# aluo7/ViT-SOM

Measured on AMD Instinct MI355X. Metric: images/sec/node ViT-SOM 40x40 CIFAR-10 bs512 (training step: fwd+bwd+all-reduce+AdamW), higher is better.
Workload: dtype f32 (Linear GEMMs on bf16 MFMA: forward from an exact 3xbf16 operand split, six products; weight / input gradients from a 2xbf16 split, three products, rel. error 4e-6)

## Files before the change

include/vitsom_hip.h:

```cpp
#ifndef VITSOM_HIP_H
#define VITSOM_HIP_H

#include <stddef.h>
#include <stdint.h>

#ifdef __cplusplus
extern "C" {
#endif

typedef struct ihipStream_t* vsom_stream_t;

#define VSOM_OK 0
#define VSOM_EINVAL (-1)
#define VSOM_EALIGN (-2)
#define VSOM_EUNSUPPORTED (-3)
#define VSOM_EWORKSPACE (-4)

#define VSOM_VERSION 100

#define VSOM_DIST_COSINE 0
#define VSOM_DIST_EUCLIDEAN 1
#define VSOM_DIST_MANHATTAN 2

int vsom_version(void);
// ... 70 lines not shown
                               const float* gamma, const float* resid, float* dX, int rows, int cols, void* part,
                               size_t part_bytes, vsom_stream_t stream);
int vsom_layernorm_bwd_finish_many(const int64_t* jobs_dev, int first, int count, int max_cols, vsom_stream_t stream);

int vsom_linear_bwd_input_ln_supported(int M, int N, int K);
size_t vsom_linear_bwd_input_ln_partial_bytes(int M, int K);
int vsom_linear_bwd_input_ln(const float* dY, long lddy, const float* Wt, int M, int N, int K, const float* X,
                             const float* mean, const float* rstd, const float* gamma, const float* resid, float* dX,
                             float* dgamma, float* dbeta, void* ws, size_t ws_bytes, vsom_stream_t stream);
int vsom_linear_bwd_input_ln_partial(const float* dY, long lddy, const float* Wt, int M, int N, int K, const float* X,
                                     const float* mean, const float* rstd, const float* gamma, const float* resid,
                                     float* dX, void* part, size_t part_bytes, vsom_stream_t stream);

int vsom_attention_fwd(const float* qkv, float* out, float* lse, int B, int N, int H, int hd,
                       vsom_stream_t stream);
int vsom_attention_bwd(const float* qkv, const float* out, const float* dout, const float* lse,
                       float* dqkv, float* delta_ws, int B, int N, int H, int hd,
                       vsom_stream_t stream);
int vsom_attention_probs(const float* qkv, const float* lse, float* probs, int B, int N, int H, int hd,
                         vsom_stream_t stream);
int vsom_set_attention_fused(int fused);

int vsom_attention_q1_fwd(const float* q, const float* kv, float* o, float* lse, int B, int N, int H, int hd,
                          vsom_stream_t stream);
int vsom_attention_q1_bwd(const float* dout, const float* o, const float* lse, const float* q, const float* kv, float* dq,
                          float* dkv, int B, int N, int H, int hd, vsom_stream_t stream);
int vsom_rows_add(const float* src, long lds, float* dst, long ldd, int rows, int cols, vsom_stream_t stream);

int vsom_row_inv_norm(const float* X, long ldx, int rows, int cols, float eps, float* inv_norm,
                      vsom_stream_t stream);
// ... 263 lines not shown
```

vit_som_amd/_lib.py:

```python
import ctypes as C
import os

import torch

_HERE = os.path.dirname(os.path.abspath(__file__))
LIB_PATH = os.path.join(_HERE, "libvitsom_hip.so")

c_fp = C.c_void_p
c_stream = C.c_void_p

SIGNATURES = {
    "vsom_version": (C.c_int, []),
    "vsom_last_error_string": (C.c_char_p, []),
    "vsom_linear_fwd": (C.c_int, [c_fp, C.c_long, c_fp, c_fp, c_fp, C.c_long, C.c_int, C.c_int, C.c_int, c_stream]),
    "vsom_linear_gelu_fwd": (C.c_int, [c_fp, C.c_long, c_fp, c_fp, c_fp, c_fp, C.c_int, C.c_int, C.c_int, c_stream]),
    "vsom_linear_relu_fwd": (C.c_int, [c_fp, C.c_long, c_fp, c_fp, c_fp, c_fp, C.c_int, C.c_int, C.c_int, c_stream]),
    "vsom_l1_loss_workspace_bytes": (C.c_size_t, [C.c_long]),
    "vsom_l1_loss": (C.c_int, [c_fp, c_fp, c_fp, c_fp, C.c_float, C.c_long, c_fp, C.c_size_t, c_stream]),
    "vsom_linear_residual_fwd": (C.c_int, [c_fp, C.c_long, c_fp, c_fp, c_fp, C.c_long, C.c_int, c_fp, C.c_long,
                                           C.c_int, C.c_int, C.c_int, c_stream]),
    "vsom_linear_bwd_input": (C.c_int, [c_fp, C.c_long, c_fp, c_fp, C.c_long, C.c_int, C.c_int, C.c_int, C.c_int,
                                        c_fp, c_stream]),
    "vsom_linear_bwd_input_t": (C.c_int, [c_fp, C.c_long, c_fp, c_fp, C.c_long, C.c_int, C.c_int, C.c_int, C.c_int,
                                          c_fp, c_stream]),
# ... 10 lines not shown
                                       C.c_int, c_stream]),
    "vsom_patch_embed_bwd_workspace_bytes": (C.c_size_t, [C.c_int] * 5),
    "vsom_patch_embed_bwd": (C.c_int, [c_fp, c_fp, c_fp, c_fp, c_fp, C.c_int, C.c_int, C.c_int, C.c_int, C.c_int,
                                       c_fp, C.c_size_t, c_stream]),
    "vsom_layernorm_fwd": (C.c_int, [c_fp, c_fp, c_fp, c_fp, c_fp, c_fp, C.c_int, C.c_int, C.c_float, c_stream]),
    "vsom_layernorm_bwd_workspace_bytes": (C.c_size_t, [C.c_int, C.c_int]),
    "vsom_layernorm_bwd": (C.c_int, [c_fp] * 9 + [C.c_int, C.c_int, c_fp, C.c_size_t, c_stream]),
    "vsom_layernorm_bwd_deferrable": (C.c_int, [C.c_int, C.c_int]),
    "vsom_layernorm_bwd_partial": (C.c_int, [c_fp] * 7 + [C.c_int, C.c_int, c_fp, C.c_size_t, c_stream]),
    "vsom_layernorm_bwd_finish_many": (C.c_int, [c_fp, C.c_int, C.c_int, C.c_int, c_stream]),
    "vsom_linear_bwd_input_ln_supported": (C.c_int, [C.c_int, C.c_int, C.c_int]),
    "vsom_linear_bwd_input_ln_partial_bytes": (C.c_size_t, [C.c_int, C.c_int]),
    "vsom_linear_bwd_input_ln": (C.c_int, [c_fp, C.c_long, c_fp, C.c_int, C.c_int, C.c_int] + [c_fp] * 8 + [c_fp, C.c_size_t, c_stream]),
    "vsom_linear_bwd_input_ln_partial": (C.c_int, [c_fp, C.c_long, c_fp, C.c_int, C.c_int, C.c_int] + [c_fp] * 6 + [c_fp, C.c_size_t, c_stream]),
    "vsom_attention_fwd": (C.c_int, [c_fp, c_fp, c_fp, C.c_int, C.c_int, C.c_int, C.c_int, c_stream]),
    "vsom_attention_bwd": (C.c_int, [c_fp] * 6 + [C.c_int] * 4 + [c_stream]),
    "vsom_set_attention_fused": (C.c_int, [C.c_int]),
    "vsom_attention_probs": (C.c_int, [c_fp, c_fp, c_fp, C.c_int, C.c_int, C.c_int, C.c_int, c_stream]),
    "vsom_attention_q1_fwd": (C.c_int, [c_fp] * 4 + [C.c_int] * 4 + [c_stream]),
    "vsom_attention_q1_bwd": (C.c_int, [c_fp] * 7 + [C.c_int] * 4 + [c_stream]),
    "vsom_rows_add": (C.c_int, [c_fp, C.c_long, c_fp, C.c_long, C.c_int, C.c_int, c_stream]),
    "vsom_tape_begin": (C.c_int, []),
    "vsom_tape_cut": (C.c_int, []),
    "vsom_tape_pause": (C.c_int, [C.c_int]),
    "vsom_tape_end": (C.c_int, []),
    "vsom_tape_recording": (C.c_int, []),
    "vsom_tape_segment_ops": (C.c_int, [C.c_int, C.c_int]),
    "vsom_tape_replay": (C.c_int, [C.c_int, C.c_int]),
    "vsom_tape_destroy": (C.c_int, [C.c_int]),
    "vsom_event_record": (C.c_int, [C.c_int, c_stream]),
# ... 257 lines not shown
```

vit_som_amd/csrc/attention.hip:

```cpp
#include "common.h"
#include "attention_layout.h"

#include <atomic>

#include <stdlib.h>

#pragma clang fp contract(off)

namespace vsom {

int gemm_grad_products();

static std::atomic<int> g_attn_fused{1};

#ifdef VSOM_ATTN_STAMPS
__device__ unsigned long long* g_attn_stamps = nullptr;
#define ATTN_STAMP(i)                                                                              \
    do {                                                                                           \
        if (threadIdx.x == 0 && g_attn_stamps) g_attn_stamps[blockIdx.x * 16 + (i)] = __builtin_amdgcn_s_memrealtime(); \
    } while (0)
#define ATTN_STAMP_HWID()                                                                          \
    do {                                                                                           \
        if (threadIdx.x == 0 && g_attn_stamps) {                                                   \
            unsigned hw, xcc;                                                                      \
// ... 134 lines not shown
__device__ __forceinline__ float tile_sum(float v) {
    v += dpp_row<0x128>(v); v += dpp_row<0x124>(v); v += dpp_row<0x122>(v); v += dpp_row<0x121>(v);
    return v;
}
__device__ __forceinline__ float tile_max(float v) {
    v = fmaxf(v, dpp_row<0x128>(v)); v = fmaxf(v, dpp_row<0x124>(v));
    v = fmaxf(v, dpp_row<0x122>(v)); v = fmaxf(v, dpp_row<0x121>(v));
    return v;
}
__device__ __forceinline__ float wave_sum64(float v) { return group_sum(tile_sum(v)); }
template <bool EXTRA>
__device__ __forceinline__ int tok(int t, int r) { return (EXTRA ? 1 : 0) + 16 * t + r; }

template <int HDP>
__device__ __forceinline__ void stage_rows(float* lds, const float* __restrict__ src, long rs, int N, int nrows,
                                           int hd) {
    constexpr int S = ACfg<HDP>::S;
    if constexpr (ACfg<HDP>::VEC) {
        constexpr int C4 = HDP / 4;
        for (int idx = threadIdx.x; idx < nrows * C4; idx += blockDim.x) {
            const int row = idx / C4, c4 = idx % C4;
            f32x4 v = {0.f, 0.f, 0.f, 0.f};
            if (row < N) v = *reinterpret_cast<const f32x4*>(src + (long)row * rs + 4 * c4);
            *reinterpret_cast<f32x4*>(lds + ACfg<HDP>::off(row, 4 * c4)) = v;
        }
    } else {
        for (int idx = threadIdx.x; idx < nrows * HDP; idx += blockDim.x) {
            const int row = idx / HDP, c = idx % HDP;
            lds[row * S + c] = (row < N && c < hd) ? src[(long)row * rs + c] : 0.f;
        }
    }
}
template <int HDP>
__device__ __forceinline__ void stage_rows_pair(float* ldsA, const float* __restrict__ srcA, long rsA, float* ldsB,
                                                const float* __restrict__ srcB, long rsB, int N, int nrows, int hd) {
    if constexpr (ACfg<HDP>::VEC) {
        constexpr int C4 = HDP / 4;
        const int total = nrows * C4, step = blockDim.x;
        for (int base = threadIdx.x; base < total; base += 4 * step) {
            f32x4 va[4], vb[4];
#pragma unroll
            for (int u = 0; u < 4; ++u) {
                const int idx = base + u * step, row = idx / C4, c4 = idx % C4;
                va[u] = f32x4{0.f, 0.f, 0.f, 0.f};
                vb[u] = f32x4{0.f, 0.f, 0.f, 0.f};
                if (idx < total && row < N) {
                    va[u] = *reinterpret_cast<const f32x4*>(srcA + (long)row * rsA + 4 * c4);
                    vb[u] = *reinterpret_cast<const f32x4*>(srcB + (long)row * rsB + 4 * c4);
                }
            }
#pragma unroll
            for (int u = 0; u < 4; ++u) {
                const int idx = base + u * step, row = idx / C4, c4 = idx % C4;
                if (idx < total) {
                    *reinterpret_cast<f32x4*>(ldsA + ACfg<HDP>::off(row, 4 * c4)) = va[u];
                    *reinterpret_cast<f32x4*>(ldsB + ACfg<HDP>::off(row, 4 * c4)) = vb[u];
                }
            }
        }
    } else {
        stage_rows<HDP>(ldsA, srcA, rsA, N, nrows, hd);
        stage_rows<HDP>(ldsB, srcB, rsB, N, nrows, hd);
    }
}
template <int HDP>
__device__ __forceinline__ void stage_rows_quad(float* l0, const float* __restrict__ s0, long r0, float* l1,
                                                const float* __restrict__ s1, long r1, float* l2,
                                                const float* __restrict__ s2, long r2, float* l3,
                                                const float* __restrict__ s3, long r3, int N, int nrows) {
    constexpr int C4 = HDP / 4;
    const int total = nrows * C4, step = blockDim.x;
    for (int base = threadIdx.x; base < total; base += 4 * step) {
        f32x4 v[4][4];
#pragma unroll
        for (int u = 0; u < 4; ++u) {
            const int idx = base + u * step, row = idx / C4, c4 = idx % C4;
            const bool ok = idx < total && row < N;
// ... 4 lines not shown
            v[3][u] = ok ? *reinterpret_cast<const f32x4*>(s3 + (long)row * r3 + 4 * c4) : z;
        }
#pragma unroll
        for (int u = 0; u < 4; ++u) {
            const int idx = base + u * step, row = idx / C4, c4 = idx % C4;
            if (idx < total) {
                *reinterpret_cast<f32x4*>(l0 + ACfg<HDP>::off(row, 4 * c4)) = v[0][u];
                *reinterpret_cast<f32x4*>(l1 + ACfg<HDP>::off(row, 4 * c4)) = v[1][u];
                *reinterpret_cast<f32x4*>(l2 + ACfg<HDP>::off(row, 4 * c4)) = v[2][u];
                *reinterpret_cast<f32x4*>(l3 + ACfg<HDP>::off(row, 4 * c4)) = v[3][u];
            }
        }
    }
}
template <int HDP>
__device__ __forceinline__ void stage_vec(float* lds, const float* __restrict__ src, int hd) {
    for (int c = threadIdx.x; c < HDP; c += blockDim.x) lds[c] = (c < hd) ? src[c] : 0.f;
}

template <int HDP>
__device__ __forceinline__ void load_frag(float (&f)[ACfg<HDP>::NMM], const float* rowptr, int qp, bool ok,
                                          int hd) {
    if constexpr (ACfg<HDP>::VEC) {
#pragma unroll
        for (int g = 0; g < HDP / 16; ++g) {
            f32x4 v = {0.f, 0.f, 0.f, 0.f};
            if (ok) v = *reinterpret_cast<const f32x4*>(rowptr + 16 * g + 4 * qp);
#pragma unroll
            for (int s = 0; s < 4; ++s) f[4 * g + s] = v[s];
        }
    } else {
#pragma unroll
// ... 252 lines not shown
    for (int t = 0; t < ntile; ++t) {
        f32x4 s, dp;
        score_tile2<HDP>(Qs, tok<EXTRA>(t, 0), kf, Ds, tok<EXTRA>(t, 0), vf, r, qp, s, dp);
        f32x4 p, ds;
#pragma unroll
        for (int e = 0; e < 4; ++e) {
            const int query = tok<EXTRA>(t, 4 * qp + e);
            p[e] = (EXTRA || (query < N && kok)) ? __expf(s[e] * scale - Ls[query]) : 0.f;
            ds[e] = p[e] * (dp[e] - Es[query]) * scale;
        }
        accum_tile2<HDP>(dv, Ds, p, dk, Qs, ds, tok<EXTRA>(t, 0), r, qp);
    }
}

template <int HDP, bool EXTRA>
__global__ __launch_bounds__(512, 4) void attn_fwd_kernel(const float* __restrict__ qkv, float* __restrict__ out,
                                                       float* __restrict__ lse, int N, int H, int hd,
                                                       float scale) {
    extern __shared__ __attribute__((aligned(16))) float smem[];
    constexpr int NDT = ACfg<HDP>::NDT;
    constexpr int NMM = ACfg<HDP>::NMM;
    const int b = blockIdx.x / H, h = blockIdx.x % H;
    const int E = H * hd, E3 = 3 * E;
    const int lane = threadIdx.x & 63, wave = threadIdx.x >> 6, nwaves = blockDim.x >> 6;
    const int r = lane & 15, qp = lane >> 4;
    const AttnLayout<float*> lay(smem, N, HDP, EXTRA, nwaves, ATTN_LDS_FWD);
    const int ntile = lay.ntile;
    float* Ks = lay.Y0;
    float* Vs = lay.Y1;
    float* X0 = lay.X0;
    float* PA = lay.PA;
    const float* base = qkv + (long)b * N * E3 + h * hd;
    float qf[NMM];
    ATTN_STAMP(0);
    ATTN_STAMP_HWID();
    load_frag<HDP>(qf, base + (long)tok<EXTRA>(wave, r) * E3, qp, tok<EXTRA>(wave, r) < N, hd);
    stage_rows_pair<HDP>(Ks, base + E, E3, Vs, base + 2 * E, E3, N, lay.nrows, hd);
    if (EXTRA) stage_vec<HDP>(X0, base, hd);
    __syncthreads();
    ATTN_STAMP(1);

    float x0m = -INFINITY, x0l = 0.f, x0o = 0.f;

    for (int qt = wave; qt < ntile; qt += nwaves) {
        const int query = tok<EXTRA>(qt, r);
        const bool qok = query < N;
        if (qt != wave) load_frag<HDP>(qf, base + (long)query * E3, qp, qok, hd);
        float m = -INFINITY, l = 0.f;
        f32x4 o[NDT];
#pragma unroll
        for (int dt = 0; dt < NDT; ++dt) o[dt] = f32x4{0.f, 0.f, 0.f, 0.f};
        if (EXTRA) {
            m = frag_dot_row<HDP>(qf, Ks, qp) * scale;
// ... 71 lines not shown
        if (wave == 0) {
            float m = s00;
            for (int w = 0; w < nwaves; ++w) m = fmaxf(m, PA[w * lay.paw + HDP]);
            float l = __expf(s00 - m);
            float o = (HDP >= 64 || lane < HDP) ? l * Vs[lane] : 0.f;
            for (int w = 0; w < nwaves; ++w) {
                const float a = __expf(PA[w * lay.paw + HDP] - m);
                l = fmaf(PA[w * lay.paw + HDP + 1], a, l);
                if (HDP >= 64 || lane < HDP) o = fmaf(PA[w * lay.paw + lane], a, o);
            }
            if (lane < hd) out[((long)b * N) * E + h * hd + lane] = o / l;
            if (lane == 0) lse[((long)b * H + h) * N] = m + logf(l);
        }
    }
    ATTN_STAMP(3);
}

template <int HDP, bool EXTRA>
__global__ __launch_bounds__(512) void attn_bwd_dq_kernel(const float* __restrict__ qkv,
                                                          const float* __restrict__ out,
                                                          const float* __restrict__ dout,
                                                          const float* __restrict__ lse,
                                                          float* __restrict__ dqkv, float* __restrict__ delta,
                                                          int N, int H, int hd, float scale) {
    extern __shared__ __attribute__((aligned(16))) float smem[];
    constexpr int NDT = ACfg<HDP>::NDT;
    constexpr int NMM = ACfg<HDP>::NMM;
    const int b = blockIdx.x / H, h = blockIdx.x % H;
    const int E = H * hd, E3 = 3 * E;
    const int lane = threadIdx.x & 63, wave = threadIdx.x >> 6, nwaves = blockDim.x >> 6;
// ... 488 lines not shown
    if (hd <= 8) return 8;
    return 0;
}
static size_t attn_lds_bytes(int N, int hdp, AttnLds kind) {
    return AttnLayout<size_t>(0, N, hdp, use_extra(N), attn_waves(N), kind).end * sizeof(float);
}
static size_t attn_shared_lds_bytes(int N, int hdp) { return attn_lds_bytes(N, hdp, ATTN_LDS_FUSED) + 2 * hdp * sizeof(float); }

template <int HDP, bool EXTRA>
static int launch_fwd_t(const float* qkv, float* out, float* lse, int B, int N, int H, int hd, hipStream_t st) {
    const size_t lds = attn_lds_bytes(N, HDP, ATTN_LDS_FWD);
    VSOM_LAUNCH((attn_fwd_kernel<HDP, EXTRA>), dim3(B * H), dim3(64 * attn_waves(N)), lds, st, qkv, out, lse, N, H, hd,
                       1.0f / sqrtf((float)hd));
    return launch_status("attn_fwd_kernel");
}
enum AttnBwd : int { ATTN_BWD_TWO_LAUNCH = 0, ATTN_BWD_FUSED = 1, ATTN_BWD_SHARED = 2, ATTN_BWD_SHARED_BF16X3 = 3 };
static AttnBwd attn_bwd_plan(int N, int hdp, int hook, int grad_products) {
    const bool vec = hdp % 16 == 0;
    const AttnLayout<size_t> fused(0, N, hdp, use_extra(N), attn_waves(N), ATTN_LDS_FUSED);
    const int nt = fused.ntile, nrows = fused.nrows;
    if (vec && (hook == 1 || hook == 3) && nt <= 4 && attn_waves(N) == nt && 16 * nt * (16 * nt + 4) <= nrows * (hdp + 4) &&
        attn_shared_lds_bytes(N, hdp) <= 80 * 1024)
        return (hdp == 64 && grad_products == 3 && hook == 1) ? ATTN_BWD_SHARED_BF16X3 : ATTN_BWD_SHARED;
    if (vec && hook != 0 && fused.end * sizeof(float) <= 80 * 1024) return ATTN_BWD_FUSED;
    return ATTN_BWD_TWO_LAUNCH;
}

int attn_bwd_threads(int N) { return 64 * attn_waves(N); }
int attn_bwd_plan_now(int N, int hd) {
    const int hdp = attn_hdp(hd);
// ... 108 lines not shown
int vsom_attention_fwd(const float* qkv, float* out, float* lse, int B, int N, int H, int hd, vsom_stream_t stream) {
    VSOM_REQUIRE(qkv && out && lse, VSOM_EINVAL, "attention_fwd: null pointer");
    int hdp;
    int rc = attn_check("attention_fwd", B, N, H, hd, &hdp);
    if (rc) return rc;
    VSOM_REQUIRE(hdp % 16 != 0 || (aligned16(qkv) && aligned16(out)), VSOM_EALIGN, "attention_fwd: 16-byte alignment required");
    switch (hdp) {
        case 4: return launch_fwd<4>(qkv, out, lse, B, N, H, hd, stream);
        case 8: return launch_fwd<8>(qkv, out, lse, B, N, H, hd, stream);
        case 16: return launch_fwd<16>(qkv, out, lse, B, N, H, hd, stream);
        case 32: return launch_fwd<32>(qkv, out, lse, B, N, H, hd, stream);
        default: return launch_fwd<64>(qkv, out, lse, B, N, H, hd, stream);
    }
}

int vsom_attention_bwd(const float* qkv, const float* out, const float* dout, const float* lse, float* dqkv,
                       float* delta_ws, int B, int N, int H, int hd, vsom_stream_t stream) {
    VSOM_REQUIRE(qkv && out && dout && lse && dqkv && delta_ws, VSOM_EINVAL, "attention_bwd: null pointer");
    int hdp;
    int rc = attn_check("attention_bwd", B, N, H, hd, &hdp);
    if (rc) return rc;
    VSOM_REQUIRE(hdp % 16 != 0 || (aligned16(qkv) && aligned16(out) && aligned16(dout) && aligned16(dqkv)), VSOM_EALIGN,
                 "attention_bwd: 16-byte alignment required");
    switch (hdp) {
        case 4: return launch_bwd<4>(qkv, out, dout, lse, dqkv, delta_ws, B, N, H, hd, stream);
        case 8: return launch_bwd<8>(qkv, out, dout, lse, dqkv, delta_ws, B, N, H, hd, stream);
        case 16: return launch_bwd<16>(qkv, out, dout, lse, dqkv, delta_ws, B, N, H, hd, stream);
        case 32: return launch_bwd<32>(qkv, out, dout, lse, dqkv, delta_ws, B, N, H, hd, stream);
        default: return launch_bwd<64>(qkv, out, dout, lse, dqkv, delta_ws, B, N, H, hd, stream);
    }
// ... 12 lines not shown
```

vit_som_amd/csrc/layernorm.hip:

```cpp
#include "gemm_f32.h"
#include "layernorm_bwd.h"

namespace vsom {

template <int MAXV>
__global__ __launch_bounds__(256) void layernorm_fwd_kernel(const float* __restrict__ X,
                                                            const float* __restrict__ gamma,
                                                            const float* __restrict__ beta,
                                                            float* __restrict__ Y, float* __restrict__ mean,
                                                            float* __restrict__ rstd, int rows, int cols,
                                                            float eps) {
    const int lane = threadIdx.x & 63;
    const int row = blockIdx.x * 4 + (threadIdx.x >> 6);
    if (row >= rows) return;
    const float* x = X + (long)row * cols;
    float v[MAXV];
    float s = 0.f;
#pragma unroll
    for (int j = 0; j < MAXV; ++j) {
        const int c = lane + 64 * j;
        v[j] = (c < cols) ? x[c] : 0.f;
        s += v[j];
    }
    const float mu = wave_sum(s) / (float)cols;
// ... 78 lines not shown
}


template <int NCH>
__global__ __launch_bounds__(256) void layernorm_fwd_v4_kernel(const float* __restrict__ X, const float* __restrict__ gamma,
                                                               const float* __restrict__ beta, float* __restrict__ Y,
                                                               float* __restrict__ mean, float* __restrict__ rstd, int rows,
                                                               int cols, float eps) {
    const int sub = threadIdx.x & 15;
    const int row = blockIdx.x * 16 + (threadIdx.x >> 4);
    const bool ok = row < rows;
    const f32x4* x = reinterpret_cast<const f32x4*>(X + (long)(ok ? row : 0) * cols);
    const float inv_n = 1.0f / (float)cols;
    f32x4 v[NCH];
    bool cv[NCH];
    float s = 0.f;
#pragma unroll
    for (int j = 0; j < NCH; ++j) {
        cv[j] = 4 * (sub + 16 * j) < cols;
        v[j] = cv[j] ? x[sub + 16 * j] : f32x4{0.f, 0.f, 0.f, 0.f};
        s += (v[j][0] + v[j][1]) + (v[j][2] + v[j][3]);
    }
    const float mu = group16_sum(s) * inv_n;
    float q = 0.f;
#pragma unroll
    for (int j = 0; j < NCH; ++j)
#pragma unroll
        for (int e = 0; e < 4; ++e) { const float d = cv[j] ? v[j][e] - mu : 0.f; q = fmaf(d, d, q); }
    const float rs = rsqrtf(group16_sum(q) * inv_n + eps);
    if (!ok) return;
    f32x4* y = reinterpret_cast<f32x4*>(Y + (long)row * cols);
#pragma unroll
    for (int j = 0; j < NCH; ++j) {
        if (!cv[j]) continue;
        const f32x4 g4 = reinterpret_cast<const f32x4*>(gamma)[sub + 16 * j];
        const f32x4 b4 = reinterpret_cast<const f32x4*>(beta)[sub + 16 * j];
        f32x4 o;
#pragma unroll
        for (int e = 0; e < 4; ++e) o[e] = (v[j][e] - mu) * rs * g4[e] + b4[e];
        y[sub + 16 * j] = o;
    }
    if (sub == 0) { mean[row] = mu; rstd[row] = rs; }
}

template <int NCH>
__global__ __launch_bounds__(256) void layernorm_bwd_v4_kernel(const float* __restrict__ dY, const float* __restrict__ X,
                                                               const float* __restrict__ mean, const float* __restrict__ rstd,
                                                               const float* __restrict__ gamma, const float* __restrict__ resid,
                                                               float* __restrict__ dX, float* __restrict__ part, int rows,
                                                               int cols) {
    __shared__ __attribute__((aligned(16))) float sh[16 * 2 * 64 * NCH];
    const int sub = threadIdx.x & 15, rg = threadIdx.x >> 4;
    const float inv_n = 1.0f / (float)cols;
    f32x4 gam[NCH], dg[NCH], db[NCH];
    bool cv[NCH];
// ... 160 lines not shown
```

vit_som_amd/ops.py:

```python
from contextlib import contextmanager
from typing import Optional

import torch

from . import _lib as _lib_mod
from ._lib import check, lib, ptr, stream

_scratch = {}
_retired = []

_timers = {}


def enable_timer(name: str):
    _timers[name] = []


def disable_timers():
    _timers.clear()


def timer_ms(name: str):
    ev = _timers.get(name, [])
    if not ev:
# ... 120 lines not shown
    return dx


def transpose_many(src_base, dst_base, table, max_rows, max_cols):
    _f32(src_base, "src_base"); _f32(dst_base, "dst_base")
    assert table.dtype == torch.int64 and table.is_contiguous() and table.ndim == 2 and table.shape[1] == 4
    assert table.device == src_base.device == dst_base.device
    check(lib.vsom_transpose_many(ptr(src_base), ptr(dst_base), table.data_ptr(), table.shape[0], int(max_rows),
                                  int(max_cols), stream()), "vsom_transpose_many")
    return dst_base


GEMM_F32, GEMM_SPLIT_BF16, GEMM_SPLIT_BF16_GRAD3 = 0, 1, 2


def set_gemm_mode(mode: int):
    check(lib.vsom_set_gemm_mode(int(mode)), "vsom_set_gemm_mode")


def get_gemm_mode() -> int:
    return int(lib.vsom_get_gemm_mode())


def set_wgrad_tiles(mode):
    global _wgrad_tiles
    check(lib.vsom_set_wgrad_tiles(int(mode)), "vsom_set_wgrad_tiles")
    _wgrad_tiles = int(mode)


_wgrad_tiles = 2


# ... 140 lines not shown
    check(lib.vsom_linear_bwd_input_ln(*args, ptr(dgamma), ptr(dbeta), ptr(ws), ws.numel(), stream()), "vsom_linear_bwd_input_ln")
    return dx


def linear_bwd_input_ln_partial(dy, Wt, x, mean, rstd, gamma, resid, dx, part):
    args = _ln_fused_args(dy, Wt, x, mean, rstd, gamma, resid, dx)
    check(lib.vsom_linear_bwd_input_ln_partial(*args, ptr(part), part.numel(), stream()), "vsom_linear_bwd_input_ln_partial")
    return dx


def attention_fwd(qkv, out, lse, B, N, H, hd):
    assert qkv.is_contiguous() and out.is_contiguous() and lse.is_contiguous()
    _f32(qkv, "qkv")
    check(lib.vsom_attention_fwd(ptr(qkv), ptr(out), ptr(lse), B, N, H, hd, stream()), "vsom_attention_fwd")
    return out


def attention_bwd(qkv, out, dout, lse, dqkv, delta, B, N, H, hd):
    assert all(t.is_contiguous() for t in (qkv, out, dout, lse, dqkv, delta))
    check(lib.vsom_attention_bwd(ptr(qkv), ptr(out), ptr(dout), ptr(lse), ptr(dqkv), ptr(delta), B, N, H, hd, stream()),
          "vsom_attention_bwd")
    return dqkv


def attention_probs(qkv, lse, probs, B, N, H, hd):
    assert qkv.is_contiguous() and lse.is_contiguous() and probs.is_contiguous() and probs.shape == (B, H, N, N)
    _f32(qkv, "qkv"); _f32(probs, "probs")
    check(lib.vsom_attention_probs(ptr(qkv), ptr(lse), ptr(probs), B, N, H, hd, stream()), "vsom_attention_probs")
    return probs

# ... 1130 lines not shown
```

vit_som_amd/tuning.py:

```python


class _Hooks:
    side_stream = True
    fwd_split = True
    fwd_split_blocks = None
    overlap_allreduce = True
    bucket_blocks = 3
    bmu_planes = True
    adamw_planes = False
    ln_reduce_batched = True
    bmu_overlap = False
    launch_tape = True
    cls_prune = True
    ln_bwd_fused = True

    def set(self, **kw):
        for k, v in kw.items():
            if not hasattr(_Hooks, k):
                raise AttributeError(f"unknown hook {k!r}")
            setattr(self, k, v)
        return self

    def signature(self):
        return tuple((k, getattr(self, k)) for k in sorted(vars(_Hooks)) if not k.startswith("_") and not callable(getattr(_Hooks, k)))

    def reset(self):
        for k in list(self.__dict__):
            delattr(self, k)
        return self
# ... 4 lines not shown
```

vit_som_amd/vit.py:

```python
import math
from typing import Dict

import numpy as np
import torch
import torch.nn as nn

from . import ops
from ._base import _Acts
from ._lib import Event, on_stream
from .tuning import hooks


def _sincos_1d(embed_dim: int, pos: np.ndarray) -> np.ndarray:
    omega = np.arange(embed_dim // 2, dtype=np.float64) / (embed_dim / 2.0)
    omega = 1.0 / 10000 ** omega
    out = np.einsum("m,d->md", pos.reshape(-1).astype(np.float64), omega)
    return np.concatenate([np.sin(out), np.cos(out)], axis=1)


def get_2d_sincos_pos_embed(embed_dim: int, grid_size: int, cls_token: bool = False) -> np.ndarray:
    gh = np.arange(grid_size, dtype=np.float32)
    gw = np.arange(grid_size, dtype=np.float32)
    grid = np.stack(np.meshgrid(gw, gh), axis=0).reshape(2, 1, grid_size, grid_size)
    emb = np.concatenate([_sincos_1d(embed_dim // 2, grid[0]), _sincos_1d(embed_dim // 2, grid[1])], axis=1)
    if cls_token:
# ... 212 lines not shown
        Hd = max([b.hidden for b in self.blocks] + [b.hidden for b in self.decoder_blocks])
        a.g = [f(T * W) for _ in range(5)]
        a.dh2, a.dqkv2, a.da = [f(T * Hd), f(T * Hd)], [f(T * 3 * W), f(T * 3 * W)], f(T * W)
        a.delta = f(B * max(self.num_heads, self.decoder_num_heads) * N)
        a.dpred = f(T, pd)
        a.d_xe = f(T, E)
        a.version = 0
        keep = list(self._acts.items())[-1:]
        self._acts = dict(keep + [(B, a)])
        return a

    def _block_fwd(self, blk: Block, L: _Acts, x_in: torch.Tensor, B: int, N: int):
        T = B * N
        ops.layernorm_fwd(x_in, blk.norm1.weight, blk.norm1.bias, L.a1, L.mean1, L.rstd1, self.eps)
        ops.linear_fwd(L.a1, blk.attn.qkv.weight, blk.attn.qkv.bias, L.qkv)
        ops.attention_fwd(L.qkv, L.ao, L.lse, B, N, blk.heads, blk.dim // blk.heads)
        ops.linear_residual_fwd(L.ao, blk.attn.proj.weight, blk.attn.proj.bias, x_in, T, L.x1)
        ops.layernorm_fwd(L.x1, blk.norm2.weight, blk.norm2.bias, L.a2, L.mean2, L.rstd2, self.eps)
        ops.linear_gelu_fwd(L.a2, blk.mlp["0"].weight, blk.mlp["0"].bias, L.hpre, L.hact)
        ops.linear_residual_fwd(L.hact, blk.mlp["2"].weight, blk.mlp["2"].bias, L.x1, T, L.x2)
        return L.x2

    def _encode(self, x: torch.Tensor, a: _Acts, side=None):
        cur = self._encode_trunk(x, a, len(self.blocks), side)
        ops.layernorm_fwd(cur, self.norm.weight, self.norm.bias, a.xe, a.mean_e, a.rstd_e, self.eps)
        return a.xe

    def _encode_trunk(self, x: torch.Tensor, a: _Acts, depth: int, side=None):
        E = self.embed_dim
        p = self.patch_embed.patch_size[0]
        a.version += 1
        ops.patch_embed_fwd(x, self.patch_embed.proj.weight.view(E, -1), self.patch_embed.proj.bias, self.pos_embed[0],
                            self.cls_token.view(E), a.tok0, a.xp, p)
# ... 293 lines not shown
```

Measured before the change: 58650.

## Fuse attention forward, output projection, residual and LayerNorm into one kernel

Adds a per-image kernel that runs attention for all three heads as wave groups, then does the output-projection GEMM from the attention output using the 3xbf16 MFMA split, adds bias and residual, and applies the following LayerNorm, all in one launch. It targets the launch overhead of three separate kernels and the global-memory round trips of the attention output and x1 between them. It only applies when H=3, hd=64, N<=96, batch>=128 and the GEMM mode is not plain f32. The cost is one block per image with a large LDS footprint, which may limit occupancy. The LayerNorm stats and apply code are moved into a shared header, with fp contraction turned off.

```diff
diff --git a/include/vitsom_hip.h b/include/vitsom_hip.h
--- a/include/vitsom_hip.h
+++ b/include/vitsom_hip.h
@@ -108,6 +108,9 @@
 
 int vsom_attention_fwd(const float* qkv, float* out, float* lse, int B, int N, int H, int hd,
                        vsom_stream_t stream);
+int vsom_attention_proj_ln_fwd(const float* qkv, const float* W, const float* b, const float* x_in, float* ao, float* lse,
+                               float* x1, const float* gamma, const float* beta, float* a2, float* mean, float* rstd, int B,
+                               int N, int H, int hd, float eps, vsom_stream_t stream);
 int vsom_attention_bwd(const float* qkv, const float* out, const float* dout, const float* lse,
                        float* dqkv, float* delta_ws, int B, int N, int H, int hd,
                        vsom_stream_t stream);
diff --git a/vit_som_amd/_lib.py b/vit_som_amd/_lib.py
--- a/vit_som_amd/_lib.py
+++ b/vit_som_amd/_lib.py
@@ -48,6 +48,7 @@
     "vsom_linear_bwd_input_ln": (C.c_int, [c_fp, C.c_long, c_fp, C.c_int, C.c_int, C.c_int] + [c_fp] * 8 + [c_fp, C.c_size_t, c_stream]),
     "vsom_linear_bwd_input_ln_partial": (C.c_int, [c_fp, C.c_long, c_fp, C.c_int, C.c_int, C.c_int] + [c_fp] * 6 + [c_fp, C.c_size_t, c_stream]),
     "vsom_attention_fwd": (C.c_int, [c_fp, c_fp, c_fp, C.c_int, C.c_int, C.c_int, C.c_int, c_stream]),
+    "vsom_attention_proj_ln_fwd": (C.c_int, [c_fp] * 12 + [C.c_int] * 4 + [C.c_float, c_stream]),
     "vsom_attention_bwd": (C.c_int, [c_fp] * 6 + [C.c_int] * 4 + [c_stream]),
     "vsom_set_attention_fused": (C.c_int, [C.c_int]),
     "vsom_attention_probs": (C.c_int, [c_fp, c_fp, c_fp, C.c_int, C.c_int, C.c_int, C.c_int, c_stream]),
diff --git a/vit_som_amd/csrc/attention.hip b/vit_som_amd/csrc/attention.hip
--- a/vit_som_amd/csrc/attention.hip
+++ b/vit_som_amd/csrc/attention.hip
@@ -1,5 +1,7 @@
 #include "common.h"
 #include "attention_layout.h"
+#include "gemm_x6.h"
+#include "layernorm_fwd.h"
 
 #include <atomic>
 
@@ -172,18 +174,18 @@
 
 template <int HDP>
 __device__ __forceinline__ void stage_rows(float* lds, const float* __restrict__ src, long rs, int N, int nrows,
-                                           int hd) {
+                                           int hd, unsigned tid = threadIdx.x, unsigned nthr = blockDim.x) {
     constexpr int S = ACfg<HDP>::S;
     if constexpr (ACfg<HDP>::VEC) {
         constexpr int C4 = HDP / 4;
-        for (int idx = threadIdx.x; idx < nrows * C4; idx += blockDim.x) {
+        for (int idx = tid; idx < nrows * C4; idx += nthr) {
             const int row = idx / C4, c4 = idx % C4;
             f32x4 v = {0.f, 0.f, 0.f, 0.f};
             if (row < N) v = *reinterpret_cast<const f32x4*>(src + (long)row * rs + 4 * c4);
             *reinterpret_cast<f32x4*>(lds + ACfg<HDP>::off(row, 4 * c4)) = v;
         }
     } else {
-        for (int idx = threadIdx.x; idx < nrows * HDP; idx += blockDim.x) {
+        for (int idx = tid; idx < nrows * HDP; idx += nthr) {
             const int row = idx / HDP, c = idx % HDP;
             lds[row * S + c] = (row < N && c < hd) ? src[(long)row * rs + c] : 0.f;
         }
@@ -191,11 +193,12 @@
 }
 template <int HDP>
 __device__ __forceinline__ void stage_rows_pair(float* ldsA, const float* __restrict__ srcA, long rsA, float* ldsB,
-                                                const float* __restrict__ srcB, long rsB, int N, int nrows, int hd) {
+                                                const float* __restrict__ srcB, long rsB, int N, int nrows, int hd,
+                                                unsigned tid = threadIdx.x, unsigned nthr = blockDim.x) {
     if constexpr (ACfg<HDP>::VEC) {
         constexpr int C4 = HDP / 4;
-        const int total = nrows * C4, step = blockDim.x;
-        for (int base = threadIdx.x; base < total; base += 4 * step) {
+        const int total = nrows * C4, step = nthr;
+        for (int base = tid; base < total; base += 4 * step) {
             f32x4 va[4], vb[4];
 #pragma unroll
             for (int u = 0; u < 4; ++u) {
@@ -217,8 +220,8 @@
             }
         }
     } else {
-        stage_rows<HDP>(ldsA, srcA, rsA, N, nrows, hd);
-        stage_rows<HDP>(ldsB, srcB, rsB, N, nrows, hd);
+        stage_rows<HDP>(ldsA, srcA, rsA, N, nrows, hd, tid, nthr);
+        stage_rows<HDP>(ldsB, srcB, rsB, N, nrows, hd, tid, nthr);
     }
 }
 template <int HDP>
@@ -253,8 +256,9 @@
     }
 }
 template <int HDP>
-__device__ __forceinline__ void stage_vec(float* lds, const float* __restrict__ src, int hd) {
-    for (int c = threadIdx.x; c < HDP; c += blockDim.x) lds[c] = (c < hd) ? src[c] : 0.f;
+__device__ __forceinline__ void stage_vec(float* lds, const float* __restrict__ src, int hd, unsigned tid = threadIdx.x,
+                                          unsigned nthr = blockDim.x) {
+    for (int c = tid; c < HDP; c += nthr) lds[c] = (c < hd) ? src[c] : 0.f;
 }
 
 template <int HDP>
@@ -537,15 +541,13 @@
 }
 
 template <int HDP, bool EXTRA>
-__global__ __launch_bounds__(512, 4) void attn_fwd_kernel(const float* __restrict__ qkv, float* __restrict__ out,
-                                                       float* __restrict__ lse, int N, int H, int hd,
-                                                       float scale) {
-    extern __shared__ __attribute__((aligned(16))) float smem[];
+__device__ __forceinline__ void attn_fwd_body(const float* __restrict__ qkv, float* __restrict__ out, float* __restrict__ lse,
+                                              int N, int H, int hd, float scale, int b, int h, int wave, int nwaves, unsigned tid, unsigned nthr,
+                                              float* smem) {
     constexpr int NDT = ACfg<HDP>::NDT;
     constexpr int NMM = ACfg<HDP>::NMM;
-    const int b = blockIdx.x / H, h = blockIdx.x % H;
     const int E = H * hd, E3 = 3 * E;
-    const int lane = threadIdx.x & 63, wave = threadIdx.x >> 6, nwaves = blockDim.x >> 6;
+    const int lane = threadIdx.x & 63;
     const int r = lane & 15, qp = lane >> 4;
     const AttnLayout<float*> lay(smem, N, HDP, EXTRA, nwaves, ATTN_LDS_FWD);
     const int ntile = lay.ntile;
@@ -558,8 +560,8 @@
     ATTN_STAMP(0);
     ATTN_STAMP_HWID();
     load_frag<HDP>(qf, base + (long)tok<EXTRA>(wave, r) * E3, qp, tok<EXTRA>(wave, r) < N, hd);
-    stage_rows_pair<HDP>(Ks, base + E, E3, Vs, base + 2 * E, E3, N, lay.nrows, hd);
-    if (EXTRA) stage_vec<HDP>(X0, base, hd);
+    stage_rows_pair<HDP>(Ks, base + E, E3, Vs, base + 2 * E, E3, N, lay.nrows, hd, tid, nthr);
+    if (EXTRA) stage_vec<HDP>(X0, base, hd, tid, nthr);
     __syncthreads();
     ATTN_STAMP(1);
 
@@ -661,6 +663,147 @@
         }
     }
     ATTN_STAMP(3);
+}
+
+template <int HDP, bool EXTRA>
+__global__ __launch_bounds__(512, 4) void attn_fwd_kernel(const float* __restrict__ qkv, float* __restrict__ out,
+                                                       float* __restrict__ lse, int N, int H, int hd,
+                                                       float scale) {
+    extern __shared__ __attribute__((aligned(16))) float smem[];
+    attn_fwd_body<HDP, EXTRA>(qkv, out, lse, N, H, hd, scale, blockIdx.x / H, blockIdx.x % H, threadIdx.x >> 6, blockDim.x >> 6,
+                              threadIdx.x, blockDim.x, smem);
+}
+
+template <int WPG>
+struct AttnProjCfg {
+    static constexpr int H = 3, HDP = 64, E = H * HDP;
+    static constexpr int NW = H * WPG, NT = NW * 64;
+    static constexpr int NRB = WPG == 1 ? 1 : WPG <= 3 ? 2 : 3;
+    static constexpr int BM = 96, BN = E, WN = 3;
+    static constexpr int NCG = BN / (32 * WN), NCW = NRB * NCG;
+    static constexpr int NTS = WPG == 1 ? 192 : WPG <= 3 ? 384 : 768;
+    static constexpr int PA = BM * X6_RS, PB = BN * X6_RS, ST = 3 * (PA + PB);
+    static constexpr int STAGES = 2;
+    static constexpr int LROW = BN + 8;
+    static constexpr int TILE_BYTES = NRB * 32 * LROW * 4;
+    static constexpr int NCH = E / 64;
+    static_assert(NCW <= NW && NTS <= NT && BM % (NTS / 8) == 0 && BN % (NTS / 8) == 0, "attn_proj_ln_kernel geometry");
+};
+
+template <bool EXTRA, int WPG>
+__global__ __launch_bounds__(AttnProjCfg<WPG>::NT) void attn_proj_ln_kernel(
+    const float* __restrict__ qkv, const float* __restrict__ W, const float* __restrict__ bias, const float* __restrict__ x_in,
+    float* ao, float* __restrict__ lse, float* __restrict__ x1, const float* __restrict__ gamma, const float* __restrict__ beta,
+    float* __restrict__ a2, float* __restrict__ mean, float* __restrict__ rstd, int N, float scale, float eps, int group_floats) {
+    using Cfg = AttnProjCfg<WPG>;
+    constexpr int E = Cfg::E, NT = Cfg::NT, NTS = Cfg::NTS, BM = Cfg::BM, BN = Cfg::BN, WN = Cfg::WN, NCH = Cfg::NCH;
+    constexpr int PA = Cfg::PA, PB = Cfg::PB, LROW = Cfg::LROW;
+    extern __shared__ __attribute__((aligned(16))) float smem[];
+    const int t = threadIdx.x, lane = t & 63, wave = t >> 6;
+    const int b = blockIdx.x;
+
+    {
+        const int g = wave / WPG;
+        attn_fwd_body<Cfg::HDP, EXTRA>(qkv, ao, lse, N, Cfg::H, Cfg::HDP, scale, b, g, wave - g * WPG, WPG, t - g * (WPG * 64),
+                                       WPG * 64, smem + g * group_floats);
+    }
+    __syncthreads();
+
+    char* As = reinterpret_cast<char*>(smem);
+    char* Bs = As + 3 * PA;
+    const int r = lane & 31, h = lane >> 5;
+    const bool computes = wave < Cfg::NCW;
+    const int wm0 = (wave / Cfg::NCG) * 32, wn0 = (wave % Cfg::NCG) * (WN * 32);
+    f32x16 acc[WN];
+#pragma unroll
+    for (int j = 0; j < WN; ++j)
+#pragma unroll
+        for (int v = 0; v < 16; ++v) acc[j][v] = 0.f;
+    {
+        const bool stages = NTS == NT || t < NTS;
+        const __amdgpu_buffer_rsrc_t rsA = __builtin_amdgcn_make_buffer_rsrc(ao + (long)b * N * E, 0, N * E * 4, 0x00020000);
+        const __amdgpu_buffer_rsrc_t rsB = __builtin_amdgcn_make_buffer_rsrc(const_cast<float*>(W), 0, E * E * 4, 0x00020000);
+        StageRegs<BM, NTS> sa;
+        StageRegs<BN, NTS> sb;
+        OffKC<BM, NTS> oa;
+        OffKC<BN, NTS> ob;
+        init_kc<BM, NTS>(oa, E, 0, N, t);
+        init_kc<BN, NTS>(ob, E, 0, E, t);
+        auto gload = [&](int kt) {
+            if (stages) {
+                load_kc_fast<BM, NTS>(sa, rsA, oa, kt << 5, E, t);
+                load_kc_fast<BN, NTS>(sb, rsB, ob, kt << 5, E, t);
+            }
+        };
+        auto lstore = [&](int so) {
+            if (stages) {
+                x6_store<BM, 3, NTS>(sa, As + so, t);
+                x6_store<BN, 3, NTS>(sb, Bs + so, t);
+            }
+        };
+        auto mfma_tile = [&](int so) {
+            if (computes) {
+#pragma unroll
+                for (int ks = 0; ks < 2; ++ks) {
+                    bf16x8 a[3], bq[WN][3];
+#pragma unroll
+                    for (int pl = 0; pl < 3; ++pl)
+                        a[pl] = *reinterpret_cast<const bf16x8*>(As + so + pl * PA + x6_chunk_off(wm0 + r, 2 * ks + h));
+#pragma unroll
+                    for (int j = 0; j < WN; ++j)
+#pragma unroll
+                        for (int pl = 0; pl < 3; ++pl)
+                            bq[j][pl] = *reinterpret_cast<const bf16x8*>(Bs + so + pl * PB + x6_chunk_off(wn0 + j * 32 + r, 2 * ks + h));
+#pragma unroll
+                    for (int j = 0; j < WN; ++j) x6_products<3>(acc[j], a, bq[j]);
+                }
+            }
+        };
+        X6_KLOOP(Cfg::STAGES, Cfg::ST, 0, E / 32, gload, lstore, mfma_tile);
+    }
+    __syncthreads();
+    float* st = smem;
+    if (computes) {
+#pragma unroll
+        for (int j = 0; j < WN; ++j)
+#pragma unroll
+            for (int v = 0; v < 16; ++v) st[(wm0 + (v & 3) + 8 * (v >> 2) + 4 * h) * LROW + wn0 + j * 32 + r] = acc[j][v];
+    }
+    __syncthreads();
+
+    const int sub = t & 15, rg = t >> 4;
+    const bool norm = a2 != nullptr;
+    const float inv_n = 1.0f / (float)E;
+    const f32x4 zero = {0.f, 0.f, 0.f, 0.f};
+    f32x4 bia[NCH], gam[NCH], bet[NCH];
+    bool cv[NCH];
+#pragma unroll
+    for (int j = 0; j < NCH; ++j) {
+        cv[j] = true;
+        bia[j] = bias ? reinterpret_cast<const f32x4*>(bias)[sub + 16 * j] : zero;
+        gam[j] = norm ? reinterpret_cast<const f32x4*>(gamma)[sub + 16 * j] : zero;
+        bet[j] = norm ? reinterpret_cast<const f32x4*>(beta)[sub + 16 * j] : zero;
+    }
+    for (int row = rg; row < N; row += NT / 16) {
+        const long grow = (long)b * N + row;
+        f32x4 v[NCH];
+#pragma unroll
+        for (int j = 0; j < NCH; ++j) {
+            const f32x4 rr = reinterpret_cast<const f32x4*>(x_in + grow * E)[sub + 16 * j];
+            const f32x4 a = *reinterpret_cast<const f32x4*>(st + row * LROW + 4 * (sub + 16 * j));
+#pragma unroll
+            for (int e = 0; e < 4; ++e) v[j][e] = a[e] + bia[j][e] + rr[e];
+        }
+#pragma unroll
+        for (int j = 0; j < NCH; ++j) reinterpret_cast<f32x4*>(x1 + grow * E)[sub + 16 * j] = v[j];
+        if (norm) {
+            float mu, rs;
+            ln_fwd_stats<NCH>(v, cv, inv_n, eps, mu, rs);
+#pragma unroll
+            for (int j = 0; j < NCH; ++j) reinterpret_cast<f32x4*>(a2 + grow * E)[sub + 16 * j] = ln_fwd_apply(v[j], mu, rs, gam[j], bet[j]);
+            if (sub == 0) { mean[grow] = mu; rstd[grow] = rs; }
+        }
+    }
 }
 
 template <int HDP, bool EXTRA>
@@ -1179,6 +1322,36 @@
                        1.0f / sqrtf((float)hd));
     return launch_status("attn_fwd_kernel");
 }
+static int attn_proj_group_floats(int N) {
+    const size_t end = AttnLayout<size_t>(0, N, 64, use_extra(N), attn_waves(N), ATTN_LDS_FWD).end;
+    return (int)((end + 3) & ~size_t(3));
+}
+template <int WPG>
+static size_t attn_proj_lds_bytes(int N) {
+    using Cfg = AttnProjCfg<WPG>;
+    size_t lds = (size_t)Cfg::H * attn_proj_group_floats(N) * sizeof(float);
+    if (lds < (size_t)Cfg::STAGES * Cfg::ST) lds = Cfg::STAGES * Cfg::ST;
+    if (lds < (size_t)Cfg::TILE_BYTES) lds = Cfg::TILE_BYTES;
+    return lds;
+}
+template <int WPG>
+static int launch_attn_proj(const float* qkv, const float* W, const float* bias, const float* x_in, float* ao, float* lse,
+                            float* x1, const float* gamma, const float* beta, float* a2, float* mean, float* rstd, int B, int N,
+                            float eps, hipStream_t st) {
+    const size_t lds = attn_proj_lds_bytes<WPG>(N);
+    VSOM_REQUIRE(lds <= 160 * 1024, VSOM_EUNSUPPORTED, "attention_proj_ln_fwd: N=%d needs %zu B of LDS (> 160 KiB)", N, lds);
+    const dim3 grid(B), block(AttnProjCfg<WPG>::NT);
+    const float scale = 1.0f / sqrtf(64.0f);
+    const int gf = attn_proj_group_floats(N);
+    if (use_extra(N))
+        VSOM_LAUNCH((attn_proj_ln_kernel<true, WPG>), grid, block, lds, st, qkv, W, bias, x_in, ao, lse, x1, gamma, beta, a2, mean,
+                    rstd, N, scale, eps, gf);
+    else
+        VSOM_LAUNCH((attn_proj_ln_kernel<false, WPG>), grid, block, lds, st, qkv, W, bias, x_in, ao, lse, x1, gamma, beta, a2, mean,
+                    rstd, N, scale, eps, gf);
+    return launch_status("attn_proj_ln_kernel");
+}
+
 enum AttnBwd : int { ATTN_BWD_TWO_LAUNCH = 0, ATTN_BWD_FUSED = 1, ATTN_BWD_SHARED = 2, ATTN_BWD_SHARED_BF16X3 = 3 };
 static AttnBwd attn_bwd_plan(int N, int hdp, int hook, int grad_products) {
     const bool vec = hdp % 16 == 0;
@@ -1317,6 +1490,28 @@
     }
 }
 
+int vsom_attention_proj_ln_fwd(const float* qkv, const float* W, const float* b, const float* x_in, float* ao, float* lse,
+                               float* x1, const float* gamma, const float* beta, float* a2, float* mean, float* rstd, int B,
+                               int N, int H, int hd, float eps, vsom_stream_t stream) {
+    VSOM_REQUIRE(qkv && W && x_in && ao && lse && x1, VSOM_EINVAL, "attention_proj_ln_fwd: null pointer");
+    const int n_ln = (gamma != nullptr) + (beta != nullptr) + (a2 != nullptr) + (mean != nullptr) + (rstd != nullptr);
+    VSOM_REQUIRE(n_ln == 0 || n_ln == 5, VSOM_EINVAL, "attention_proj_ln_fwd: LayerNorm pointers must be all set or all null");
+    VSOM_REQUIRE(B > 0 && N > 0 && H > 0 && hd > 0, VSOM_EINVAL, "attention_proj_ln_fwd: bad shape B=%d N=%d H=%d hd=%d", B, N, H, hd);
+    VSOM_REQUIRE(gemm_mode() != VSOM_GEMM_F32, VSOM_EUNSUPPORTED, "attention_proj_ln_fwd: not in VSOM_GEMM_F32 mode");
+    VSOM_REQUIRE(hd == 64, VSOM_EUNSUPPORTED, "attention_proj_ln_fwd: head dim %d not supported (64)", hd);
+    VSOM_REQUIRE((long)H * hd <= 192 && H == 3, VSOM_EUNSUPPORTED, "attention_proj_ln_fwd: E = %ld not supported (3 heads of 64)", (long)H * hd);
+    VSOM_REQUIRE(N <= 96, VSOM_EUNSUPPORTED, "attention_proj_ln_fwd: N=%d > 96", N);
+    VSOM_REQUIRE(aligned16(qkv) && aligned16(W) && (!b || aligned16(b)) && aligned16(x_in) && aligned16(ao) && aligned16(x1) &&
+                     (!n_ln || (aligned16(gamma) && aligned16(beta) && aligned16(a2))),
+                 VSOM_EALIGN, "attention_proj_ln_fwd: 16-byte alignment required");
+    switch (attn_waves(N)) {
+        case 1: return launch_attn_proj<1>(qkv, W, b, x_in, ao, lse, x1, gamma, beta, a2, mean, rstd, B, N, eps, stream);
+        case 2: return launch_attn_proj<2>(qkv, W, b, x_in, ao, lse, x1, gamma, beta, a2, mean, rstd, B, N, eps, stream);
+        case 3: return launch_attn_proj<3>(qkv, W, b, x_in, ao, lse, x1, gamma, beta, a2, mean, rstd, B, N, eps, stream);
+        default: return launch_attn_proj<4>(qkv, W, b, x_in, ao, lse, x1, gamma, beta, a2, mean, rstd, B, N, eps, stream);
+    }
+}
+
 int vsom_attention_bwd(const float* qkv, const float* out, const float* dout, const float* lse, float* dqkv,
                        float* delta_ws, int B, int N, int H, int hd, vsom_stream_t stream) {
     VSOM_REQUIRE(qkv && out && dout && lse && dqkv && delta_ws, VSOM_EINVAL, "attention_bwd: null pointer");
diff --git a/vit_som_amd/csrc/layernorm.hip b/vit_som_amd/csrc/layernorm.hip
--- a/vit_som_amd/csrc/layernorm.hip
+++ b/vit_som_amd/csrc/layernorm.hip
@@ -1,5 +1,6 @@
 #include "gemm_f32.h"
 #include "layernorm_bwd.h"
+#include "layernorm_fwd.h"
 
 namespace vsom {
 
@@ -116,20 +117,13 @@
     const float inv_n = 1.0f / (float)cols;
     f32x4 v[NCH];
     bool cv[NCH];
-    float s = 0.f;
 #pragma unroll
     for (int j = 0; j < NCH; ++j) {
         cv[j] = 4 * (sub + 16 * j) < cols;
         v[j] = cv[j] ? x[sub + 16 * j] : f32x4{0.f, 0.f, 0.f, 0.f};
-        s += (v[j][0] + v[j][1]) + (v[j][2] + v[j][3]);
-    }
-    const float mu = group16_sum(s) * inv_n;
-    float q = 0.f;
-#pragma unroll
-    for (int j = 0; j < NCH; ++j)
-#pragma unroll
-        for (int e = 0; e < 4; ++e) { const float d = cv[j] ? v[j][e] - mu : 0.f; q = fmaf(d, d, q); }
-    const float rs = rsqrtf(group16_sum(q) * inv_n + eps);
+    }
+    float mu, rs;
+    ln_fwd_stats<NCH>(v, cv, inv_n, eps, mu, rs);
     if (!ok) return;
     f32x4* y = reinterpret_cast<f32x4*>(Y + (long)row * cols);
 #pragma unroll
@@ -137,10 +131,7 @@
         if (!cv[j]) continue;
         const f32x4 g4 = reinterpret_cast<const f32x4*>(gamma)[sub + 16 * j];
         const f32x4 b4 = reinterpret_cast<const f32x4*>(beta)[sub + 16 * j];
-        f32x4 o;
-#pragma unroll
-        for (int e = 0; e < 4; ++e) o[e] = (v[j][e] - mu) * rs * g4[e] + b4[e];
-        y[sub + 16 * j] = o;
+        y[sub + 16 * j] = ln_fwd_apply(v[j], mu, rs, g4, b4);
     }
     if (sub == 0) { mean[row] = mu; rstd[row] = rs; }
 }
diff --git a/vit_som_amd/csrc/layernorm_fwd.h b/vit_som_amd/csrc/layernorm_fwd.h
--- /dev/null
+++ b/vit_som_amd/csrc/layernorm_fwd.h
@@ -0,0 +1,30 @@
+#pragma once
+#include "layernorm_bwd.h"
+
+namespace vsom {
+
+template <int NCH>
+__device__ __forceinline__ void ln_fwd_stats(const f32x4 (&v)[NCH], const bool (&cv)[NCH], float inv_n, float eps, float& mu,
+                                             float& rs) {
+#pragma clang fp contract(off)
+    float s = 0.f;
+#pragma unroll
+    for (int j = 0; j < NCH; ++j) s += (v[j][0] + v[j][1]) + (v[j][2] + v[j][3]);
+    mu = group16_sum(s) * inv_n;
+    float q = 0.f;
+#pragma unroll
+    for (int j = 0; j < NCH; ++j)
+#pragma unroll
+        for (int e = 0; e < 4; ++e) { const float d = cv[j] ? v[j][e] - mu : 0.f; q = fmaf(d, d, q); }
+    rs = rsqrtf(fmaf(group16_sum(q), inv_n, eps));
+}
+
+__device__ __forceinline__ f32x4 ln_fwd_apply(const f32x4& v, float mu, float rs, const f32x4& g4, const f32x4& b4) {
+#pragma clang fp contract(off)
+    f32x4 o;
+#pragma unroll
+    for (int e = 0; e < 4; ++e) o[e] = fmaf((v[e] - mu) * rs, g4[e], b4[e]);
+    return o;
+}
+
+}
diff --git a/vit_som_amd/ops.py b/vit_som_amd/ops.py
--- a/vit_som_amd/ops.py
+++ b/vit_som_amd/ops.py
@@ -158,8 +158,13 @@
 GEMM_F32, GEMM_SPLIT_BF16, GEMM_SPLIT_BF16_GRAD3 = 0, 1, 2
 
 
+_gemm_mode = GEMM_SPLIT_BF16_GRAD3
+
+
 def set_gemm_mode(mode: int):
+    global _gemm_mode
     check(lib.vsom_set_gemm_mode(int(mode)), "vsom_set_gemm_mode")
+    _gemm_mode = int(mode)
 
 
 def get_gemm_mode() -> int:
@@ -330,6 +335,25 @@
     _f32(qkv, "qkv")
     check(lib.vsom_attention_fwd(ptr(qkv), ptr(out), ptr(lse), B, N, H, hd, stream()), "vsom_attention_fwd")
     return out
+
+
+def attention_proj_ln_supported(N, H, hd) -> bool:
+    return H == 3 and hd == 64 and 0 < N <= 96 and _gemm_mode != GEMM_F32
+
+
+def attention_proj_ln_fwd(qkv, W, bias, x_in, ao, lse, x1, B, N, H, hd, gamma=None, beta=None, a2=None, mean=None, rstd=None,
+                          eps=1e-6):
+    E = H * hd
+    assert all(t.is_contiguous() for t in (qkv, W, x_in, ao, lse, x1))
+    _f32(qkv, "qkv"); _f32(W, "W"); _f32(x_in, "x_in"); _f32(x1, "x1")
+    assert qkv.shape == (B * N, 3 * E) and W.shape == (E, E) and x_in.shape == (B * N, E) == x1.shape == ao.shape
+    assert lse.numel() == B * H * N
+    if a2 is not None:
+        assert a2.is_contiguous() and a2.shape == x1.shape and mean.numel() == B * N == rstd.numel()
+    check(lib.vsom_attention_proj_ln_fwd(ptr(qkv), ptr(W), ptr(bias), ptr(x_in), ptr(ao), ptr(lse), ptr(x1), ptr(gamma), ptr(beta),
+                                         ptr(a2), ptr(mean), ptr(rstd), B, N, H, hd, float(eps), stream()),
+          "vsom_attention_proj_ln_fwd")
+    return x1
 
 
 def attention_bwd(qkv, out, dout, lse, dqkv, delta, B, N, H, hd):
diff --git a/vit_som_amd/tuning.py b/vit_som_amd/tuning.py
--- a/vit_som_amd/tuning.py
+++ b/vit_som_amd/tuning.py
@@ -13,6 +13,7 @@
     launch_tape = True
     cls_prune = True
     ln_bwd_fused = True
+    attn_proj_fused = True
 
     def set(self, **kw):
         for k, v in kw.items():
diff --git a/vit_som_amd/vit.py b/vit_som_amd/vit.py
--- a/vit_som_amd/vit.py
+++ b/vit_som_amd/vit.py
@@ -9,6 +9,8 @@
 from ._base import _Acts
 from ._lib import Event, on_stream
 from .tuning import hooks
+
+ATTN_PROJ_MIN_IMAGES = 128
 
 
 def _sincos_1d(embed_dim: int, pos: np.ndarray) -> np.ndarray:
@@ -251,9 +253,14 @@
         T = B * N
         ops.layernorm_fwd(x_in, blk.norm1.weight, blk.norm1.bias, L.a1, L.mean1, L.rstd1, self.eps)
         ops.linear_fwd(L.a1, blk.attn.qkv.weight, blk.attn.qkv.bias, L.qkv)
-        ops.attention_fwd(L.qkv, L.ao, L.lse, B, N, blk.heads, blk.dim // blk.heads)
-        ops.linear_residual_fwd(L.ao, blk.attn.proj.weight, blk.attn.proj.bias, x_in, T, L.x1)
-        ops.layernorm_fwd(L.x1, blk.norm2.weight, blk.norm2.bias, L.a2, L.mean2, L.rstd2, self.eps)
+        H, hd = blk.heads, blk.dim // blk.heads
+        if hooks.attn_proj_fused and B >= ATTN_PROJ_MIN_IMAGES and ops.attention_proj_ln_supported(N, H, hd):
+            ops.attention_proj_ln_fwd(L.qkv, blk.attn.proj.weight, blk.attn.proj.bias, x_in, L.ao, L.lse, L.x1, B, N, H, hd,
+                                      blk.norm2.weight, blk.norm2.bias, L.a2, L.mean2, L.rstd2, self.eps)
+        else:
+            ops.attention_fwd(L.qkv, L.ao, L.lse, B, N, H, hd)
+            ops.linear_residual_fwd(L.ao, blk.attn.proj.weight, blk.attn.proj.bias, x_in, T, L.x1)
+            ops.layernorm_fwd(L.x1, blk.norm2.weight, blk.norm2.bias, L.a2, L.mean2, L.rstd2, self.eps)
         ops.linear_gelu_fwd(L.a2, blk.mlp["0"].weight, blk.mlp["0"].bias, L.hpre, L.hact)
         ops.linear_residual_fwd(L.hact, blk.mlp["2"].weight, blk.mlp["2"].bias, L.x1, T, L.x2)
         return L.x2
```

New measurement: 58920, median of 3. About the same (+0.5%).
